# rfahrn/RadVLM

Hardware: AMD Instinct MI355X
Metric: train image-instruction pairs/sec, LLaVA-1.5-7B 336px (higher is better)
Workload: dtype bf16; 1 GPU; llava15_7b full fine-tune step (ViT frozen): fwd+bwd+AdamW, S=704, 32 pairs/GPU/step; global_batch=32, seq_len=704, parallelism=dp1, rows_with_a_label_only=last layer's o_proj / norm / MLP, final norm, lm_head, cross entropy

## Files before the change

radvlm_amd/csrc/gemm_bf16.hip:

```cpp
#include <type_traits>
#include "common.h"
#include "radvlm_hip.h"
#include "gemm_plan.h"
#include <stdlib.h>

namespace {

constexpr int BM = 128, BN = 128, BK = 64;
constexpr int STAGE_BYTES = (BM + BN) * BK * 2;
constexpr int NSTAGE = 2;

struct GemmParams {
    const bf16* A; const bf16* B; void* C; const bf16* bias; const void* R; const bf16* zeros;
    long lda, ldb, ldc, ldr;
    int M, N, K, act, out_f32, res_f32, tiles_m, tiles_n;
    float alpha;
    const bf16* A2; const bf16* B2; long lda2, ldb2; int K2;
    float* ws; int splits;
    int n_full;
    int pgrid;
    const float* rope_cs; const int* rope_pos; int rope_S, rope_cols, rope_hd;
    int F; bf16* C2; long ldc2; const bf16* G; long ldg;
    unsigned bytesA, bytesB;
    unsigned bytesA2, bytesB2;
// ... 532 lines not shown
                if (full) {
                    const f32x4 r0 = *(const f32x4*)rp, r1 = *(const f32x4*)(rp + 4);
#pragma unroll
                    for (int r = 0; r < 4; ++r) { v[r] += r0[r]; v[4 + r] += r1[r]; }
                } else {
#pragma unroll
                    for (int r = 0; r < 8; ++r) if (r < nv) v[r] += rp[r];
                }
            } else {
                const bf16* rp = (const bf16*)P.R + (long)m * P.ldr + n;
                if (full) {
                    const bf16x8 rr = *(const bf16x8*)rp;
#pragma unroll
                    for (int r = 0; r < 8; ++r) v[r] += bf2f(rr[r]);
                } else {
#pragma unroll
                    for (int r = 0; r < 8; ++r) if (r < nv) v[r] += bf2f(rp[r]);
                }
            }
        }
        if (P.out_f32) {
            float* cp = (float*)P.C + (long)m * P.ldc + n;
            if (full) { *(f32x4*)cp = f32x4{v[0], v[1], v[2], v[3]}; *(f32x4*)(cp + 4) = f32x4{v[4], v[5], v[6], v[7]}; }
            else {
#pragma unroll
                for (int r = 0; r < 8; ++r) if (r < nv) cp[r] = v[r];
            }
        } else {
            bf16* cp = (bf16*)P.C + (long)m * P.ldc + n;
            if (full) *(bf16x8*)cp = bf16x8{f2bf(v[0]), f2bf(v[1]), f2bf(v[2]), f2bf(v[3]), f2bf(v[4]), f2bf(v[5]), f2bf(v[6]), f2bf(v[7])};
            else {
#pragma unroll
                for (int r = 0; r < 8; ++r) if (r < nv) cp[r] = f2bf(v[r]);
            }
        }
    });
}

DEVINL float rbf16(float x) { return bf2f(f2bf(x)); }
DEVINL void store8(bf16* p, const float (&v)[8]) {
    *(bf16x8*)p = bf16x8{f2bf(v[0]), f2bf(v[1]), f2bf(v[2]), f2bf(v[3]), f2bf(v[4]), f2bf(v[5]), f2bf(v[6]), f2bf(v[7])};
}

template <int EPI>
DEVINL void epilogue_fused(const f32x4 (&acc)[8][4], const GemmParams& P, int m0, int tn, int wr, int wc, int lane) {
    const int q = lane >> 4;
    static_for<8>([&](auto ii) {
        constexpr int i = decltype(ii)::value;
        const int m = m0 + wr * 128 + i * 16 + (lane & 15);
        if (m >= P.M) return;
        float lo[8] = {acc[i][0][0], acc[i][0][1], acc[i][0][2], acc[i][0][3], acc[i][1][0], acc[i][1][1], acc[i][1][2], acc[i][1][3]};
        float hi[8] = {acc[i][2][0], acc[i][2][1], acc[i][2][2], acc[i][2][3], acc[i][3][0], acc[i][3][1], acc[i][3][2], acc[i][3][3]};
        if (EPI == EPI_ROPE) {
            const int half = P.rope_hd >> 1;
            int nlo, e0;
            if (P.rope_hd == 128) { e0 = 32 * (wc & 1) + 8 * q; nlo = tn * BN2 + (wc >> 1) * 128 + e0; }
            else { e0 = 8 * q; nlo = tn * BN2 + wc * 64 + e0; }
            const int nhi = nlo + half;
            if (nlo >= P.N) return;
            if (P.bias) {
                const bf16x8 b0 = *(const bf16x8*)(P.bias + nlo), b1 = *(const bf16x8*)(P.bias + nhi);
#pragma unroll
                for (int r = 0; r < 8; ++r) { lo[r] += bf2f(b0[r]); hi[r] += bf2f(b1[r]); }
            }
            if (nlo < P.rope_cols) {
                const int pos = P.rope_pos ? P.rope_pos[m] : (m % P.rope_S);
                const float* cs = P.rope_cs + ((long)pos * half + e0) * 2;
#pragma unroll
                for (int r4 = 0; r4 < 4; ++r4) {
                    const f32x4 t = *(const f32x4*)(cs + 4 * r4);
#pragma unroll
                    for (int u = 0; u < 2; ++u) {
                        const int r = 2 * r4 + u;
                        const float co = t[2 * u], si = t[2 * u + 1];
                        const float a = rbf16(lo[r]), b = rbf16(hi[r]);
                        lo[r] = a * co - b * si;
                        hi[r] = b * co + a * si;
                    }
                }
            }
            bf16* cp = (bf16*)P.C + (long)m * P.ldc;
            store8(cp + nlo, lo);
            store8(cp + nhi, hi);
        } else if (EPI == EPI_SWIGLU_FWD) {
            const int f = tn * 128 + 32 * wc + 8 * q;
            if (f >= P.F) return;
            float a[8];
#pragma unroll
            for (int r = 0; r < 8; ++r) {
                const float g = rbf16(lo[r]), u = rbf16(hi[r]);
                a[r] = rbf16(g / (1.f + __expf(-g))) * u;
            }
            bf16* gp = (bf16*)P.C + (long)m * P.ldc;
            store8(gp + f, lo);
            store8(gp + P.F + f, hi);
            store8(P.C2 + (long)m * P.ldc2 + f, a);
        }
    });
    if (EPI == EPI_SWIGLU_BWD) {
        auto dswiglu = [&](const f32x4& x0, const f32x4& x1, const bf16x8& gv, const bf16x8& uv, bf16* cp_g, bf16* cp_u) {
            const float da[8] = {x0[0], x0[1], x0[2], x0[3], x1[0], x1[1], x1[2], x1[3]};
            float dg[8], du[8];
#pragma unroll
            for (int r = 0; r < 8; ++r) {
                const float g = bf2f(gv[r]), u = bf2f(uv[r]), d = rbf16(da[r]);
                const float sg = __builtin_amdgcn_rcpf(1.f + __expf(-g));
                du[r] = d * (g * sg);
                dg[r] = d * u * (sg * (1.f + g * (1.f - sg)));
            }
            store8(cp_g, dg);
            store8(cp_u, du);
        };
        if (m0 + BM2 <= P.M && tn * BN2 + BN2 <= P.F) {
            const bf16* gp = P.G + (long)(m0 + wr * 128 + (lane & 15)) * P.ldg + tn * BN2 + wc * 64 + 8 * q;
            bf16* cp = (bf16*)P.C + (long)(m0 + wr * 128 + (lane & 15)) * P.ldc + tn * BN2 + wc * 64 + 8 * q;
            bf16x8 gq[2][4], uq[2][4];
            auto fetch = [&](int bi, bf16x8 (&gd)[4], bf16x8 (&ud)[4]) {
#pragma unroll
                for (int u = 0; u < 4; ++u) {
                    const int ia = bi * 4 + u, i = ia >> 1, a = ia & 1;
                    const bf16* p = gp + (long)i * 16 * P.ldg + 32 * a;
                    gd[u] = *(const bf16x8*)p;
                    ud[u] = *(const bf16x8*)(p + P.F);
                }
            };
            fetch(0, gq[0], uq[0]);
            static_for<4>([&](auto bt) {
                constexpr int bi = decltype(bt)::value;
                if constexpr (bi + 1 < 4) fetch(bi + 1, gq[(bi + 1) & 1], uq[(bi + 1) & 1]);
                static_for<4>([&](auto ut) {
                    constexpr int u = decltype(ut)::value, ia = bi * 4 + u, i = ia >> 1, a = ia & 1;
                    bf16* c = cp + (long)i * 16 * P.ldc + 32 * a;
                    dswiglu(acc[i][2 * a], acc[i][2 * a + 1], gq[bi & 1][u], uq[bi & 1][u], c, c + P.F);
                });
            });
            return;
        }
        static_for<16>([&](auto ia) {
            constexpr int i = decltype(ia)::value >> 1, a = decltype(ia)::value & 1;
            const int m = m0 + wr * 128 + i * 16 + (lane & 15);
            const int n = tn * BN2 + wc * 64 + 32 * a + 8 * q;
            if (m >= P.M || n >= P.F) return;
            const bf16x8 gv = *(const bf16x8*)(P.G + (long)m * P.ldg + n), uv = *(const bf16x8*)(P.G + (long)m * P.ldg + P.F + n);
            bf16* cp = (bf16*)P.C + (long)m * P.ldc;
            dswiglu(acc[i][2 * a], acc[i][2 * a + 1], gv, uv, cp + n, cp + P.F + n);
        });
    }
}

#ifdef RV_STAMPS
static long long* g_stamp_host = nullptr;
extern "C" int rv_debug_set_stamp_buffer(void* p) { g_stamp_host = (long long*)p; return 0; }
#define RV_STAMP(i) do { if (MODE == 0 && P.ws && threadIdx.x == 0) ((long long*)P.ws)[(long)blockIdx.x * 4 + (i)] = wall_clock64(); } while (0)
#else
#define RV_STAMP(i) do { } while (0)
#endif

template <bool TA, bool TB, int MODE, int EPI = EPI_NONE, bool BUF = false>
__global__ __launch_bounds__(512, 1) void gemm_kernel_256(GemmParams P) {
    extern __shared__ __attribute__((aligned(16))) char smem[];
    const int wid = wave_id(), lane = lane_id();
    const int wr = wid >> 2, wc = wid & 3;
    RV_STAMP(0);

    const int nwg = P.tiles_m * P.tiles_n;
    constexpr bool PERSIST = (MODE == 0 || MODE == 1 || MODE == 3) && BUF;
    int vtile = blockIdx.x, kslice = 0;
    bool sliced = MODE == 2;
    if (MODE == 2) { vtile = (int)blockIdx.x / P.splits; kslice = (int)blockIdx.x % P.splits; }
    if (MODE == 3 && (int)blockIdx.x >= (PERSIST ? P.pgrid : P.n_full)) {
        const int r = (int)blockIdx.x - (PERSIST ? P.pgrid : P.n_full);
        vtile = P.n_full + r / P.splits; kslice = r % P.splits; sliced = true;
    }
    int m0, n0, tn;
    auto coords = [&](int vt) {
        const int pid = xcd_remap(vt, nwg);
        constexpr int GROUP_M = RV_GROUP_M;
        const int per_group = GROUP_M * P.tiles_n;
        const int group = pid / per_group;
        const int first_m = group * GROUP_M;
        const int gsz = min(P.tiles_m - first_m, GROUP_M);
        tn = (pid % per_group) / gsz;
        m0 = (first_m + (pid % per_group) % gsz) * BM2;
        n0 = tn * BN2;
    };
    coords(vtile);

    f32x4 acc[8][4];

    const int nt1 = (P.K + BK - 1) / BK;
    const int t0 = sliced ? (int)((long)kslice * nt1 / P.splits) : 0;
    const int nt = sliced ? (int)((long)(kslice + 1) * nt1 / P.splits) - t0 : (MODE == 1 ? nt1 + (P.K2 + BK - 1) / BK : nt1);
    __amdgpu_buffer_rsrc_t rsA, rsB;
    HalfPlan plA[2], plB[2];
    if constexpr (BUF) {
        rsA = __builtin_amdgcn_make_buffer_rsrc((void*)P.A, 0, P.bytesA, 0x00020000);
        rsB = __builtin_amdgcn_make_buffer_rsrc((void*)P.B, 0, P.bytesB, 0x00020000);
    }
    auto make_plans = [&]() {
#pragma unroll
        for (int h = 0; h < 2; ++h) {
            plA[h] = plan_half<TA, false, 0>(P.lda, m0 + h * 128, P.M, wid, lane, h, 0, P.bytesA);
            if (EPI == EPI_ROPE) plB[h] = P.rope_hd == 128 ? plan_half<TB, true, 1>(P.ldb, n0 + h * 128, P.N, wid, lane, h, 0, P.bytesB)
                                                            : plan_half<TB, true, 0>(P.ldb, n0 + h * 128, P.N, wid, lane, h, 0, P.bytesB);
            else if (EPI == EPI_SWIGLU_FWD) plB[h] = plan_half<TB, true, 2>(P.ldb, tn * 128, P.N, wid, lane, h, P.F, P.bytesB);
            else plB[h] = plan_half<TB, true, 0>(P.ldb, n0 + h * 128, P.N, wid, lane, h, 0, P.bytesB);
        }
    };
    __amdgpu_buffer_rsrc_t rsA2, rsB2;
    HalfPlan plA2[2], plB2[2];
    if constexpr (BUF && MODE == 1) {
        rsA2 = __builtin_amdgcn_make_buffer_rsrc((void*)P.A2, 0, P.bytesA2, 0x00020000);
        rsB2 = __builtin_amdgcn_make_buffer_rsrc((void*)P.B2, 0, P.bytesB2, 0x00020000);
    }
    auto make_plans2 = [&]() {
#pragma unroll
        for (int h = 0; h < 2; ++h) {
            plA2[h] = plan_half<TA, false, 0>(P.lda2, m0 + h * 128, P.M, wid, lane, h, 0, P.bytesA2);
            plB2[h] = plan_half<TB, true, 0>(P.ldb2, n0 + h * 128, P.N, wid, lane, h, 0, P.bytesB2);
        }
    };
    if constexpr (BUF) make_plans();
    if constexpr (BUF && MODE == 1) make_plans2();
    const int kstepA = TA ? (int)(P.lda * BK * 2) : BK * 2, kstepB = TB ? (int)(P.ldb * BK * 2) : BK * 2;
    const int kstepA2 = TA ? (int)(P.lda2 * BK * 2) : BK * 2, kstepB2 = TB ? (int)(P.ldb2 * BK * 2) : BK * 2;
    auto stageA = [&](int t, int slot, int h, auto pair_tag) {
        constexpr int PAIR = decltype(pair_tag)::value;
        char* dst = smem + (slot * 2 + h) * HALF_BYTES;
        if constexpr (BUF) {
            if (MODE == 1 && (PAIR == 1 || (PAIR == 2 && t >= nt1))) stage_half_buf(rsA2, plA2[h], (t - nt1) * kstepA2, dst, wid);
            else stage_half_buf(rsA, plA[h], (t0 + t) * kstepA, dst, wid);
            return;
        }
        if (MODE == 1 && t >= nt1) stage_half<TA>(P.A2, P.lda2, m0 + h * 128, P.M, (t - nt1) * BK, P.K2, P.zeros, dst, wid, lane);
        else stage_half<TA>(P.A, P.lda, m0 + h * 128, P.M, (t0 + t) * BK, P.K, P.zeros, dst, wid, lane);
    };
    auto stageB = [&](int t, int h, auto pair_tag) {
        constexpr int PAIR = decltype(pair_tag)::value;
        char* dst = smem + B_RING_OFF + ((t & 1) * 2 + h) * HALF_BYTES;
        if constexpr (BUF) {
            if (MODE == 1 && (PAIR == 1 || (PAIR == 2 && t >= nt1))) stage_half_buf(rsB2, plB2[h], (t - nt1) * kstepB2, dst, wid);
            else stage_half_buf(rsB, plB[h], (t0 + t) * kstepB, dst, wid);
            return;
        }
        if (MODE == 1 && t >= nt1) stage_half<TB, true>(P.B2, P.ldb2, n0 + h * 128, P.N, (t - nt1) * BK, P.K2, P.zeros, dst, wid, lane);
        else if (EPI == EPI_ROPE) {
            if (P.rope_hd == 128) stage_half<TB, true, 1>(P.B, P.ldb, n0 + h * 128, P.N, (t0 + t) * BK, P.K, P.zeros, dst, wid, lane);
            else stage_half<TB, true>(P.B, P.ldb, n0 + h * 128, P.N, (t0 + t) * BK, P.K, P.zeros, dst, wid, lane);
        } else if (EPI == EPI_SWIGLU_FWD) stage_half<TB, true, 2>(P.B, P.ldb, tn * 128, P.N, (t0 + t) * BK, P.K, P.zeros, dst, wid, lane, h, P.F);
        else stage_half<TB, true>(P.B, P.ldb, n0 + h * 128, P.N, (t0 + t) * BK, P.K, P.zeros, dst, wid, lane);
    };

    constexpr std::integral_constant<int, 0> P0{};
    constexpr std::integral_constant<int, 1> P1{};
    constexpr std::integral_constant<int, 2> PR{};
    stageA(0, 0, 0, P0); stageA(0, 0, 1, P0); stageB(0, 0, P0); stageB(0, 1, P0);
    int vt0 = blockIdx.x;
    do {
    if (nt > 1) { stageA(1, 1, 0, PR); stageA(1, 1, 1, PR); stageB(1, 0, PR); stageB(1, 1, PR); asm volatile("s_waitcnt vmcnt(8)" ::: "memory"); }
    else asm volatile("s_waitcnt vmcnt(0)" ::: "memory");
    __builtin_amdgcn_s_barrier();
    RV_STAMP(1);
#pragma unroll
    for (int i = 0; i < 8; ++i)
#pragma unroll
        for (int j = 0; j < 4; ++j) acc[i][j] = f32x4{0.f, 0.f, 0.f, 0.f};

    int aslot = 0;
    long long dbg[4] = {0, 0, 0, 0};
    auto step = [&](int t, auto stage_tag, auto pair_tag) {
        constexpr int STAGE = decltype(stage_tag)::value;
        const char* At = smem + (aslot * 2 + wr) * HALF_BYTES;
        const char* Bt = smem + B_RING_OFF + ((t & 1) * 2 + (wc >> 1)) * HALF_BYTES;
        const int aslot2 = aslot == 0 ? 2 : aslot - 1;
        const int brow0 = (wc & 1) * 64;
        ktile_256<TA, TB>(acc, At, Bt, brow0, lane,
                          [&]() { if (STAGE == 1 || (STAGE == 2 && t + 2 < nt)) stageA(t + 2, aslot2, 0, pair_tag); },
                          [&]() { if (STAGE == 1 || (STAGE == 2 && t + 2 < nt)) stageA(t + 2, aslot2, 1, pair_tag); },
                          [&]() { if (STAGE == 1 || (STAGE == 2 && t + 2 < nt)) stageB(t + 2, 0, pair_tag); },
                          [&]() { if (STAGE == 1 || (STAGE == 2 && t + 2 < nt)) stageB(t + 2, 1, pair_tag); }, dbg);
        RV_ACC_BEGIN();
        if (STAGE == 1 || (STAGE == 2 && t + 2 < nt)) asm volatile("s_waitcnt vmcnt(8)" ::: "memory");
        else asm volatile("s_waitcnt vmcnt(0)" ::: "memory");
        RV_ACC_END(1);
        aslot = aslot == 2 ? 0 : aslot + 1;
        RV_ACC_BEGIN();
        BAR_LGKM();
        RV_ACC_END(2);
    };
    if constexpr ((MODE == 2 || MODE == 1) && !BUF) {
        for (int t = 0; t < nt; ++t) step(t, std::integral_constant<int, 2>{}, PR);
    } else if constexpr (MODE == 1) {
        int t = 0;
        for (; t + 2 < nt1; ++t) step(t, std::integral_constant<int, 1>{}, P0);
        for (; t + 2 < nt; ++t) step(t, std::integral_constant<int, 1>{}, P1);
        for (; t < nt; ++t) step(t, std::integral_constant<int, 0>{}, P0);
    } else {
        int t = 0;
        for (; t + 2 < nt; ++t) step(t, std::integral_constant<int, 1>{}, P0);
        for (; t < nt; ++t) step(t, std::integral_constant<int, 0>{}, P0);
    }
#ifdef RV_STAMPS
    if (MODE == 0 && P.ws && lane == 0) {
        long long* o = (long long*)P.ws + (long)gridDim.x * 4 + ((long)blockIdx.x * 8 + wid) * 3;
        o[0] = dbg[0]; o[1] = dbg[1]; o[2] = dbg[2];
    }
#endif

    RV_STAMP(2);
    if (MODE == 3 && sliced) {
        float* slab = P.ws + ((long)(vtile - P.n_full) * P.splits + kslice) * (BM2 * BN2);
#pragma unroll
        for (int i = 0; i < 8; ++i)
#pragma unroll
            for (int a = 0; a < 2; ++a) {
                float* wp = slab + (wr * 128 + i * 16 + (lane & 15)) * BN2 + wc * 64 + 32 * a + 8 * (lane >> 4);
                *(f32x4*)wp = acc[i][2 * a];
                *(f32x4*)(wp + 4) = acc[i][2 * a + 1];
            }
        return;
    }
    const int m0e = m0, n0e = n0, tne = tn;
    bool more = false;
    if constexpr (PERSIST) {
        vt0 += MODE == 3 ? P.pgrid : (int)gridDim.x;
        more = !sliced && vt0 < (MODE == 3 ? P.n_full : nwg);
        if (more) {
            coords(vt0); make_plans();
            if constexpr (MODE == 1) make_plans2();
            stageA(0, 0, 0, P0); stageA(0, 0, 1, P0); stageB(0, 0, P0); stageB(0, 1, P0);
        }
    }
    if (EPI != EPI_NONE) epilogue_fused<EPI>(acc, P, m0e, tne, wr, wc, lane);
    else epilogue_256<MODE == 3 ? 0 : MODE>(acc, P, m0e, n0e, wr, wc, lane, kslice);
#ifdef RV_STAMPS
    asm volatile("s_waitcnt vmcnt(0)" ::: "memory");
#endif
    RV_STAMP(3);
    if (!more) break;
    } while (PERSIST);
}

__global__ void splitk_reduce_kernel(GemmParams P) {
    const long i = (long)blockIdx.x * blockDim.x + threadIdx.x;
    const long total = (long)P.M * P.N;
    if (i >= total) return;
    const int m = (int)(i / P.N), n = (int)(i % P.N);
    float s = 0.f;
    for (int k = 0; k < P.splits; ++k) s += P.ws[(long)k * total + i];
    s *= P.alpha;
    if (P.bias) s += bf2f(P.bias[n]);
    s = apply_act(s, P.act);
    if (P.R) s += P.res_f32 ? ((const float*)P.R)[(long)m * P.ldr + n] : bf2f(((const bf16*)P.R)[(long)m * P.ldr + n]);
    if (P.out_f32) ((float*)P.C)[(long)m * P.ldc + n] = s;
    else ((bf16*)P.C)[(long)m * P.ldc + n] = f2bf(s);
}

constexpr int AG_BM = 64, AG_BN = 128;
constexpr int AG_XB = AG_BM * AG_BN * 2, AG_TB = AG_BM * 64 * 2, AG_STAGE = AG_XB + AG_TB;
struct LoraAGradParams {
    const bf16* X; const bf16* T; float* ws;
    long ldx, ldt;
    int M, R, K, splits;
    unsigned thr; unsigned long long seed;
};
DEVINL int sw128(int m) { return (((m >> 1) & 1) | (((m >> 3) & 1) << 1)) << 1; }
DEVINL bf16x8 tr_read16(const char* a, const char* b) {
    const s16x4 lo = __builtin_amdgcn_ds_read_tr16_b64_v4i16((__attribute__((address_space(3))) s16x4*)a);
    const s16x4 hi = __builtin_amdgcn_ds_read_tr16_b64_v4i16((__attribute__((address_space(3))) s16x4*)b);
    const s16x8 r = {lo[0], lo[1], lo[2], lo[3], hi[0], hi[1], hi[2], hi[3]};
    return __builtin_bit_cast(bf16x8, r);
}
__global__ __launch_bounds__(256, 3) void lora_agrad_kernel(LoraAGradParams P) {
    __shared__ __attribute__((aligned(16))) char smem[2 * AG_STAGE];
    const int wid = wave_id(), lane = lane_id(), tid = (int)threadIdx.x;
    const int ncb = (P.K + AG_BN - 1) / AG_BN;
    const int cb = (int)blockIdx.x % ncb, split = (int)blockIdx.x / ncb;
    const int c0 = cb * AG_BN;
    const int nst = (P.M + AG_BM - 1) / AG_BM;
    const int s0 = (int)((long)split * nst / P.splits), s1 = (int)((long)(split + 1) * nst / P.splits);
    const int xr = tid >> 4, xc = tid & 15;
    const int tr = tid >> 3, tc = tid & 7;
    const bool xok = c0 + xc * 8 < P.K, tok = tc * 8 < P.R;
    const bf16x8 zero8 = {0, 0, 0, 0, 0, 0, 0, 0};
    bf16x8 xv0, xv1, xv2, xv3, tv0, tv1;
    auto ldx8 = [&](int m) __attribute__((always_inline)) { return (xok && m < P.M) ? *(const bf16x8*)(P.X + (long)m * P.ldx + c0 + xc * 8) : zero8; };
    auto ldt8 = [&](int m) __attribute__((always_inline)) { return (tok && m < P.M) ? *(const bf16x8*)(P.T + (long)m * P.ldt + tc * 8) : zero8; };
    auto load = [&](int s) __attribute__((always_inline)) {
        const int m0 = s * AG_BM;
        xv0 = ldx8(m0 + xr); xv1 = ldx8(m0 + xr + 16); xv2 = ldx8(m0 + xr + 32); xv3 = ldx8(m0 + xr + 48);
        tv0 = ldt8(m0 + tr); tv1 = ldt8(m0 + tr + 32);
    };
    auto put_x = [&](bf16x8 v, int m0, int row, char* st) __attribute__((always_inline)) {
        if (P.thr) {
            const unsigned keep = rv_keep8(P.seed, (unsigned long long)(m0 + row) * (unsigned long long)P.K + (unsigned long long)(c0 + xc * 8), P.thr);
#pragma unroll
            for (int j = 0; j < 8; ++j) v[j] = (keep >> j) & 1 ? v[j] : (bf16)0.f;
        }
        *(bf16x8*)(st + row * 256 + ((xc ^ tswz(row)) << 4)) = v;
    };
    auto store = [&](int s, char* st) __attribute__((always_inline)) {
        const int m0 = s * AG_BM;
        put_x(xv0, m0, xr, st); put_x(xv1, m0, xr + 16, st); put_x(xv2, m0, xr + 32, st); put_x(xv3, m0, xr + 48, st);
        *(bf16x8*)(st + AG_XB + tr * 128 + ((tc ^ sw128(tr)) << 4)) = tv0;
        *(bf16x8*)(st + AG_XB + (tr + 32) * 128 + ((tc ^ sw128(tr + 32)) << 4)) = tv1;
    };
    const int g = lane >> 4, q = (lane >> 2) & 3, pp = lane & 3;
    const int mrow = 8 * g + q;
    int xoff[2], toff[4];
#pragma unroll
    for (int j = 0; j < 2; ++j) xoff[j] = mrow * 256 + (((((wid * 32 + 16 * j) >> 3) + (pp >> 1)) ^ tswz(mrow)) << 4) + (pp & 1) * 8;
#pragma unroll
    for (int i = 0; i < 4; ++i) toff[i] = AG_XB + mrow * 128 + ((((16 * i) >> 3) + (pp >> 1)) ^ sw128(mrow)) * 16 + (pp & 1) * 8;
    f32x4 acc[4][2];
#pragma unroll
    for (int i = 0; i < 4; ++i)
#pragma unroll
        for (int j = 0; j < 2; ++j) acc[i][j] = f32x4{0.f, 0.f, 0.f, 0.f};
    if (s0 < s1) { load(s0); store(s0, smem); }
    __syncthreads();
    for (int s = s0; s < s1; ++s) {
        const char* cur = smem + ((s - s0) & 1) * AG_STAGE;
        char* nxt = smem + (((s - s0) & 1) ^ 1) * AG_STAGE;
        if (s + 1 < s1) load(s + 1);
#pragma unroll
        for (int kk = 0; kk < 2; ++kk) {
            bf16x8 b[2], a[4];
#pragma unroll
            for (int j = 0; j < 2; ++j) b[j] = tr_read16(cur + xoff[j] + kk * 8192, cur + xoff[j] + kk * 8192 + 1024);
#pragma unroll
            for (int i = 0; i < 4; ++i) a[i] = tr_read16(cur + toff[i] + kk * 4096, cur + toff[i] + kk * 4096 + 512);
#pragma unroll
            for (int i = 0; i < 4; ++i)
#pragma unroll
                for (int j = 0; j < 2; ++j) acc[i][j] = mfma16(a[i], b[j], acc[i][j]);
        }
        if (s + 1 < s1) store(s + 1, nxt);
        __syncthreads();
    }
#pragma unroll
    for (int i = 0; i < 4; ++i)
#pragma unroll
        for (int j = 0; j < 2; ++j)
#pragma unroll
            for (int r = 0; r < 4; ++r) {
                const int ar = 16 * i + 4 * g + r, col = c0 + wid * 32 + 16 * j + (lane & 15);
                if (ar < P.R && col < P.K) P.ws[((long)split * P.R + ar) * P.K + col] = acc[i][j][r];
            }
}

__global__ __launch_bounds__(256) void tail_reduce_kernel(GemmParams P) {
    const int nwg = P.tiles_m * P.tiles_n;
    const int tt = blockIdx.x >> 5;
    const int e = ((blockIdx.x & 31) * 256 + threadIdx.x) * 8;
    const int row = e >> 8, col = e & 255;
    const int pid = xcd_remap(P.n_full + tt, nwg);
    constexpr int GROUP_M = RV_GROUP_M;
    const int per_group = GROUP_M * P.tiles_n;
    const int group = pid / per_group;
    const int first_m = group * GROUP_M;
    const int gsz = min(P.tiles_m - first_m, GROUP_M);
    const int m = (first_m + (pid % per_group) % gsz) * BM2 + row;
    const int n = ((pid % per_group) / gsz) * BN2 + col;
    if (m >= P.M || n >= P.N) return;
    float v[8] = {0, 0, 0, 0, 0, 0, 0, 0};
    for (int k = 0; k < P.splits; ++k) {
        const float* sp = P.ws + ((long)tt * P.splits + k) * (BM2 * BN2) + row * BN2 + col;
        const f32x4 a = *(const f32x4*)sp, b = *(const f32x4*)(sp + 4);
#pragma unroll
        for (int r = 0; r < 4; ++r) { v[r] += a[r]; v[4 + r] += b[r]; }
    }
    const int nv = min(8, P.N - n);
    const bool vec = nv == 8 && (P.N % 8 == 0) && (P.ldc % 8 == 0) && !P.out_f32 && (!P.R || (!P.res_f32 && P.ldr % 8 == 0)) &&
                     ((((uintptr_t)P.C) | ((uintptr_t)P.R) | ((uintptr_t)P.bias)) & 15) == 0;
    if (vec) {
        float x[8];
#pragma unroll
        for (int r = 0; r < 8; ++r) x[r] = v[r] * P.alpha;
        if (P.bias) {
            const bf16x8 bb = *(const bf16x8*)(P.bias + n);
#pragma unroll
            for (int r = 0; r < 8; ++r) x[r] += bf2f(bb[r]);
        }
        if (P.act != RV_ACT_NONE) {
#pragma unroll
            for (int r = 0; r < 8; ++r) x[r] = apply_act(x[r], P.act);
        }
        if (P.R) {
            const bf16x8 rr = *(const bf16x8*)((const bf16*)P.R + (long)m * P.ldr + n);
#pragma unroll
            for (int r = 0; r < 8; ++r) x[r] += bf2f(rr[r]);
        }
// ... 12 lines not shown

}

static_assert(PLAN_TILE128 == BM && PLAN_TILE128 == BN && PLAN_TILE256 == BM2 && PLAN_TILE256 == BN2 && PLAN_BK == BK, "gemm_plan.h plans for these tiles");
static GemmConfig g_cfg;
static int g_cus_device = -1;
static int g_reserved_cus = -1;
extern "C" int rv_gemm_select_kernel(int which) {
    if (which >= 40) g_cfg.persist = which == 41;
    else if (which >= 30) g_cfg.flat = which == 30;
    else if (which >= 20) g_cfg.tail_split = which - 20;
    else g_cfg.force_kernel = which;
    return RV_OK;
}
extern "C" int rv_gemm_set_cu_budget(int total_cus, int reserved_cus) {
    int dev = -1;
    if (hipGetDevice(&dev) != hipSuccess) dev = -1;
    if (total_cus <= 0 && (dev < 0 || hipDeviceGetAttribute(&total_cus, hipDeviceAttributeMultiprocessorCount, dev) != hipSuccess)) return RV_ERR_LAUNCH;
    g_cus_device = dev;
    g_reserved_cus = reserved_cus < 0 ? 0 : reserved_cus;
    g_cfg.cus = total_cus - g_reserved_cus < 8 ? 8 : total_cus - g_reserved_cus;
    return g_cfg.cus;
}
static int gemm_config(GemmConfig& cfg) {
    static bool env_read = false;
    if (const char* e = env_read ? nullptr : getenv("RV_GEMM_KERNEL")) g_cfg.force_kernel = atoi(e);
    env_read = true;
    int dev = 0;
    if (g_cfg.cus != 0 && hipGetDevice(&dev) == hipSuccess && dev != g_cus_device) g_cfg.cus = 0;
    if (g_cfg.cus == 0) {
        const char* e = getenv("RV_GEMM_RESERVED_CUS");
        const int rc = rv_gemm_set_cu_budget(0, g_reserved_cus >= 0 ? g_reserved_cus : (e ? atoi(e) : 0));
        if (rc < 0) return rc;
    }
    cfg = g_cfg;
    return RV_OK;
}

static GemmParams gemm_params(const void* A, int64_t lda, const void* B, int64_t ldb, void* C, int64_t ldc, const void* bias, const void* residual,
                              int64_t ldr, const void* zeros16, int M, int N, int K, float alpha, int act = RV_ACT_NONE, int out_f32 = 0, int res_f32 = 0) {
    GemmParams P = {};
    P.A = (const bf16*)A; P.B = (const bf16*)B; P.C = C; P.bias = (const bf16*)bias; P.R = residual; P.zeros = (const bf16*)zeros16;
    P.lda = lda; P.ldb = ldb; P.ldc = ldc; P.ldr = ldr;
    P.M = M; P.N = N; P.K = K; P.act = act; P.out_f32 = out_f32; P.res_f32 = res_f32; P.alpha = alpha; P.splits = 1;
    return P;
}
static void launch_splitk_reduce(const GemmParams& P, hipStream_t st) {
    hipLaunchKernelGGL(splitk_reduce_kernel, dim3((unsigned)(((long)P.M * P.N + 255) / 256)), dim3(256), 0, st, P);
}
template <bool TA, bool TB, int MODE, int EPI, bool BUF>
static void launch256(GemmParams P, const GemmPlan& pl, hipStream_t st) {
    static bool attr = false;
    if (!attr) { (void)hipFuncSetAttribute((const void*)gemm_kernel_256<TA, TB, MODE, EPI, BUF>, hipFuncAttributeMaxDynamicSharedMemorySize, LDS_BYTES2); attr = true; }
    P.tiles_m = pl.tiles_m; P.tiles_n = pl.tiles_n; P.splits = pl.splits; P.n_full = pl.n_full; P.pgrid = pl.pgrid;
    P.bytesA = pl.bytesA; P.bytesB = pl.bytesB; P.bytesA2 = pl.bytesA2; P.bytesB2 = pl.bytesB2;
    hipLaunchKernelGGL((gemm_kernel_256<TA, TB, MODE, EPI, BUF>), dim3(pl.grid), dim3(512), LDS_BYTES2, st, P);
    if (MODE == 3) hipLaunchKernelGGL(tail_reduce_kernel, dim3((pl.tiles_m * pl.tiles_n - pl.n_full) * 32), dim3(256), 0, st, P);
    if (MODE == 2) launch_splitk_reduce(P, st);
}
template <class F>
static void with_bool(bool v, F f) { if (v) f(std::true_type{}); else f(std::false_type{}); }
static void launch256_plain(const GemmParams& P, const GemmPlan& pl, bool trans_a, bool trans_b, hipStream_t st) {
    with_bool(trans_a, [&](auto ta) { with_bool(trans_b, [&](auto tb) { with_bool(pl.buf != 0, [&](auto buf) {
        constexpr bool TA = decltype(ta)::value, TB = decltype(tb)::value, BUF = decltype(buf)::value;
        switch (pl.mode) {
            case 1: launch256<TA, TB, 1, EPI_NONE, BUF>(P, pl, st); break;
            case 2: launch256<TA, TB, 2, EPI_NONE, BUF>(P, pl, st); break;
            case 3: launch256<TA, TB, 3, EPI_NONE, BUF>(P, pl, st); break;
            default: launch256<TA, TB, 0, EPI_NONE, BUF>(P, pl, st);
        }
    }); }); });
}

static int gemm_ex_impl(const void* A, int64_t lda, const void* B, int64_t ldb, void* C, int64_t ldc, const void* bias,
                        const void* residual, int64_t ldr, int M, int N, int K, int trans_a, int trans_b, float alpha,
                        int act, int out_f32, int res_f32, const void* A2, int64_t lda2, const void* B2, int64_t ldb2,
                        int K2, void* workspace, int64_t workspace_bytes, const void* zeros16, void* stream, float drop_p, uint64_t drop_seed) {
    const bool ext = A2 && B2 && K2 > 0;
    const unsigned drop_thr = drop_p > 0.f ? rv_dropout_thr16(drop_p) : 0u;
    const GemmRequest rq = {M, N, K, trans_a, trans_b, lda, ldb, ext ? K2 : 0, lda2, ldb2, workspace && workspace_bytes > 0 ? workspace_bytes : 0,
                            drop_thr ? GEMM_DROPOUT : GEMM_PLAIN};
    if (!A || !B || !C || !zeros16 || !gemm_args_ok(rq)) return RV_ERR_ARG;
    if (((uintptr_t)A | (uintptr_t)B | (uintptr_t)zeros16) & 15) return RV_ERR_ARG;
    if (ext && (((uintptr_t)A2 | (uintptr_t)B2) & 15)) return RV_ERR_ARG;
    GemmConfig cfg;
    if (const int rc = gemm_config(cfg)) return rc;
    GemmParams P = gemm_params(A, lda, B, ldb, C, ldc, bias, residual, ldr, zeros16, M, N, K, alpha, act, out_f32, res_f32);
    P.A2 = (const bf16*)A2; P.B2 = (const bf16*)B2; P.lda2 = lda2; P.ldb2 = ldb2; P.K2 = rq.K2; P.ws = (float*)workspace;
    P.drop_thr = drop_thr; P.drop_scale = drop_p > 0.f ? 1.f / (1.f - drop_p) : 1.f; P.drop_seed = drop_seed;
    const GemmPlan pl = gemm_plan(rq, cfg);
    hipStream_t st = (hipStream_t)stream;
    if (pl.use256) {
#ifdef RV_STAMPS
        if (pl.mode == 0) P.ws = (float*)g_stamp_host;
#endif
        launch256_plain(P, pl, trans_a, trans_b, st);
    } else {
        static bool attr = false;
        if (!attr) { (void)hipFuncSetAttribute((const void*)gemm_nt_kernel, hipFuncAttributeMaxDynamicSharedMemorySize, NSTAGE * STAGE_BYTES); attr = true; }
        P.tiles_m = pl.tiles_m; P.tiles_n = pl.tiles_n;
        hipLaunchKernelGGL(gemm_nt_kernel, dim3(pl.grid), dim3(256), NSTAGE * STAGE_BYTES, st, P);
    }
    return rv_check_launch();
}

extern "C" int rv_gemm_bf16_ex(const void* A, int64_t lda, const void* B, int64_t ldb, void* C, int64_t ldc, const void* bias,
                               const void* residual, int64_t ldr, int M, int N, int K, int trans_a, int trans_b, float alpha,
                               int act, int out_f32, int res_f32, const void* A2, int64_t lda2, const void* B2, int64_t ldb2,
                               int K2, void* workspace, int64_t workspace_bytes, const void* zeros16, void* stream) {
    return gemm_ex_impl(A, lda, B, ldb, C, ldc, bias, residual, ldr, M, N, K, trans_a, trans_b, alpha, act, out_f32, res_f32, A2, lda2, B2, ldb2, K2,
                        workspace, workspace_bytes, zeros16, stream, 0.f, 0);
}

extern "C" int rv_gemm_plan(int M, int N, int K, int trans_a, int trans_b, int64_t lda, int64_t ldb, int K2, int64_t lda2, int64_t ldb2,
                            int64_t workspace_bytes, int kind, int32_t* out) {
    const GemmRequest rq = {M, N, K, trans_a, trans_b, lda, ldb, K2, lda2, ldb2, workspace_bytes, kind};
    if (!out || !gemm_args_ok(rq)) return RV_ERR_ARG;
    GemmConfig cfg;
    if (const int rc = gemm_config(cfg)) return rc;
    const GemmPlan pl = gemm_plan(rq, cfg);
    out[0] = pl.use256 ? 2 : 1; out[1] = pl.mode; out[2] = pl.splits; out[3] = pl.n_full; out[4] = pl.grid; out[5] = pl.buf;
    return RV_OK;
}

extern "C" int rv_gemm_dropout_add_bf16(const void* A, int64_t lda, const void* B, int64_t ldb, void* C, int64_t ldc, int M, int N, int K,
                                        int trans_b, float alpha, float p, uint64_t seed, int accumulate, const void* zeros16, void* stream) {
    if (p < 0.f || p >= 1.f || (N & 7) || (ldc & 7) || (((uintptr_t)C) & 15)) return RV_ERR_ARG;
    return gemm_ex_impl(A, lda, B, ldb, C, ldc, nullptr, accumulate ? C : nullptr, ldc, M, N, K, 0, trans_b, alpha, RV_ACT_NONE, 0, 0, nullptr, 0,
                        nullptr, 0, 0, nullptr, 0, zeros16, stream, p, seed);
}

extern "C" int rv_gemm_bf16(const void* A, int64_t lda, const void* B, int64_t ldb, void* C, int64_t ldc, const void* bias,
                            const void* residual, int64_t ldr, int M, int N, int K, int trans_a, int trans_b, float alpha,
                            int act, int out_f32, int res_f32, const void* zeros16, void* stream) {
    return rv_gemm_bf16_ex(A, lda, B, ldb, C, ldc, bias, residual, ldr, M, N, K, trans_a, trans_b, alpha, act, out_f32, res_f32,
                           nullptr, 0, nullptr, 0, 0, nullptr, 0, zeros16, stream);
}

extern "C" int rv_gemm_nt_bf16(const void* A, int64_t lda, const void* B, int64_t ldb, void* C, int64_t ldc,
                               const void* bias, const void* residual, int64_t ldr, int M, int N, int K, int act,
                               int out_f32, int res_f32, const void* zeros16, void* stream) {
    return rv_gemm_bf16(A, lda, B, ldb, C, ldc, bias, residual, ldr, M, N, K, 0, 0, 1.0f, act, out_f32, res_f32, zeros16, stream);
}

static int fused_plan(int M, int N, int K, int trans_b, int64_t lda, int64_t ldb, GemmPlan& pl) {
    const GemmRequest rq = {M, N, K, 0, trans_b, lda, ldb, 0, 0, 0, 0, GEMM_FUSED};
    GemmConfig cfg;
    if (const int rc = gemm_config(cfg)) return rc;
    pl = gemm_plan(rq, cfg);
    if (!gemm_args_ok(rq)) pl.use256 = 0;
    return RV_OK;
}
template <int EPI, bool TB>
static int launch_fused(const GemmParams& P, const GemmPlan& pl, void* stream) {
    if (((uintptr_t)P.A | (uintptr_t)P.B | (uintptr_t)P.zeros) & 15) return RV_ERR_ARG;
    if (pl.buf) launch256<false, TB, 0, EPI, true>(P, pl, (hipStream_t)stream);
    else launch256<false, TB, 0, EPI, false>(P, pl, (hipStream_t)stream);
    return rv_check_launch();
}

extern "C" int rv_gemm_rope_bf16(const void* A, int64_t lda, const void* B, int64_t ldb, void* C, int64_t ldc, const void* bias,
                                 int M, int N, int K, const float* cos_sin, const int32_t* positions, int S, int rope_heads, int hd,
                                 void* workspace, int64_t workspace_bytes, const void* zeros16, void* stream) {
    if (!A || !B || !C || !cos_sin || !zeros16 || M <= 0 || N <= 0 || K <= 0 || rope_heads <= 0 || (long)rope_heads * hd > N) return RV_ERR_ARG;
    if ((hd & 15) || (!positions && S <= 0)) return RV_ERR_ARG;
    GemmPlan pl;
    if (const int rc = fused_plan(M, N, K, 0, lda, ldb, pl)) return rc;
    const bool fused = pl.use256 && (hd == 128 || hd == 64) && (N % 8 == 0) && (ldc % 8 == 0) && (N % hd == 0) &&
                       ((((uintptr_t)C) | ((uintptr_t)bias) | ((uintptr_t)cos_sin)) & 15) == 0;
    if (!fused) {
        int rc = rv_gemm_bf16_ex(A, lda, B, ldb, C, ldc, bias, nullptr, 0, M, N, K, 0, 0, 1.f, RV_ACT_NONE, 0, 0, nullptr, 0, nullptr, 0, 0,
                                 workspace, workspace_bytes, zeros16, stream);
        if (rc != RV_OK) return rc;
        return positions ? rv_rope_inplace_pos(C, ldc, cos_sin, positions, M, rope_heads, hd, 1, 1, stream)
                         : rv_rope_inplace(C, ldc, cos_sin, M, S, rope_heads, hd, 1, 1, stream);
    }
    GemmParams P = gemm_params(A, lda, B, ldb, C, ldc, bias, nullptr, 0, zeros16, M, N, K, 1.f);
    P.rope_cs = cos_sin; P.rope_pos = positions; P.rope_S = S > 0 ? S : 1; P.rope_cols = rope_heads * hd; P.rope_hd = hd;
    return launch_fused<EPI_ROPE, false>(P, pl, stream);
}

extern "C" int rv_gemm_swiglu_fwd_bf16(const void* A, int64_t lda, const void* Wgu, int64_t ldb, void* GU, int64_t ldgu, void* ACT,
                                       int64_t ldact, int M, int F, int K, void* workspace, int64_t workspace_bytes, const void* zeros16,
                                       void* stream) {
    if (!A || !Wgu || !GU || !ACT || !zeros16 || M <= 0 || F <= 0 || K <= 0 || (F & 7) || (ldgu & 7) || (ldact & 7)) return RV_ERR_ARG;
    GemmPlan pl;
    if (const int rc = fused_plan(M, 2 * F, K, 0, lda, ldb, pl)) return rc;
    if (!pl.use256 || ((((uintptr_t)GU) | ((uintptr_t)ACT)) & 15)) {
        int rc = rv_gemm_bf16_ex(A, lda, Wgu, ldb, GU, ldgu, nullptr, nullptr, 0, M, 2 * F, K, 0, 0, 1.f, RV_ACT_NONE, 0, 0, nullptr, 0, nullptr,
                                 0, 0, workspace, workspace_bytes, zeros16, stream);
        if (rc != RV_OK) return rc;
        return rv_swiglu_fwd(GU, ldgu, ACT, ldact, M, F, stream);
    }
    GemmParams P = gemm_params(A, lda, Wgu, ldb, GU, ldgu, nullptr, nullptr, 0, zeros16, M, 2 * F, K, 1.f);
    P.F = F; P.C2 = (bf16*)ACT; P.ldc2 = ldact;
    return launch_fused<EPI_SWIGLU_FWD, false>(P, pl, stream);
}

extern "C" int rv_gemm_swiglu_bwd_bf16(const void* dY, int64_t ldy, const void* Wd, int64_t ldw, const void* GU, int64_t ldgu, void* dGU,
                                       int64_t lddgu, void* dact_scratch, int64_t ld_dact, int M, int F, int K, void* workspace,
                                       int64_t workspace_bytes, const void* zeros16, void* stream) {
    if (!dY || !Wd || !GU || !dGU || !zeros16 || M <= 0 || F <= 0 || K <= 0 || (F & 7) || (ldgu & 7) || (lddgu & 7)) return RV_ERR_ARG;
    GemmPlan pl;
    if (const int rc = fused_plan(M, F, K, 1, ldy, ldw, pl)) return rc;
    if (!pl.use256 || ((((uintptr_t)GU) | ((uintptr_t)dGU)) & 15)) {
        if (!dact_scratch || (ld_dact & 7)) return RV_ERR_ARG;
        int rc = rv_gemm_bf16_ex(dY, ldy, Wd, ldw, dact_scratch, ld_dact, nullptr, nullptr, 0, M, F, K, 0, 1, 1.f, RV_ACT_NONE, 0, 0, nullptr, 0,
                                 nullptr, 0, 0, workspace, workspace_bytes, zeros16, stream);
        if (rc != RV_OK) return rc;
        return rv_swiglu_bwd(dact_scratch, ld_dact, GU, ldgu, dGU, lddgu, M, F, stream);
    }
    GemmParams P = gemm_params(dY, ldy, Wd, ldw, dGU, lddgu, nullptr, nullptr, 0, zeros16, M, F, K, 1.f);
    P.F = F; P.G = (const bf16*)GU; P.ldg = ldgu;
    return launch_fused<EPI_SWIGLU_BWD, true>(P, pl, stream);
}

extern "C" int rv_lora_a_grad_bf16(const void* dT, int64_t ldt, const void* X, int64_t ldx, void* gA, int64_t ldg, int M, int R, int K, float p,
                                   uint64_t seed, int accumulate, void* workspace, int64_t workspace_bytes, void* stream) {
    if (!dT || !X || !gA || !workspace || M <= 0 || R <= 0 || K <= 0 || p < 0.f || p >= 1.f) return RV_ERR_ARG;
    if (R > 64 || (R & 7) || (K & 7) || (ldx & 7) || (ldt & 7) || (p > 0.f && ldx != K)) return RV_ERR_ARG;
    if ((((uintptr_t)X) | ((uintptr_t)dT)) & 15) return RV_ERR_ARG;
    const int ncb = (K + AG_BN - 1) / AG_BN, nst = (M + AG_BM - 1) / AG_BM;
    GemmConfig cfg;
    if (const int rc = gemm_config(cfg)) return rc;
    int splits = (3 * cfg.cus + ncb - 1) / ncb;
    if (splits > nst) splits = nst;
    if (splits > 32) splits = 32;
    const int64_t per = (int64_t)R * K * 4;
    if (splits > workspace_bytes / per) splits = (int)(workspace_bytes / per);
    if (splits < 1) return RV_ERR_ARG;
    LoraAGradParams Q;
    Q.X = (const bf16*)X; Q.T = (const bf16*)dT; Q.ws = (float*)workspace; Q.ldx = ldx; Q.ldt = ldt; Q.M = M; Q.R = R; Q.K = K; Q.splits = splits;
    Q.thr = rv_dropout_thr16(p); Q.seed = seed;
    hipStream_t st = (hipStream_t)stream;
    hipLaunchKernelGGL(lora_agrad_kernel, dim3((unsigned)(ncb * splits)), dim3(256), 0, st, Q);
    GemmParams P = gemm_params(nullptr, 0, nullptr, 0, gA, ldg, nullptr, accumulate ? gA : nullptr, ldg, nullptr, R, K, 0, p > 0.f ? 1.f / (1.f - p) : 1.f);
    P.splits = splits; P.ws = (float*)workspace;
    launch_splitk_reduce(P, st);
    return rv_check_launch();
}

extern "C" int rv_lora_down_bf16(const void* X, int64_t ldx, const void* A, int64_t lda, void* T, int64_t ldt, int M, int R, int K, float alpha,
                                 float p, uint64_t seed, const void* zeros16, void* stream) {
    if (!X || !A || !T || !zeros16 || M <= 0 || R <= 0 || K <= 0 || p < 0.f || p >= 1.f) return RV_ERR_ARG;
    if (R > LD_BN || (R & 3) || (K % BK) || (p > 0.f && ldx != K) || (ldx & 7) || (lda & 7) || (ldt & 3)) return RV_ERR_ARG;
    if ((((uintptr_t)X) | ((uintptr_t)A) | ((uintptr_t)zeros16)) & 15) return RV_ERR_ARG;
    if (((uintptr_t)T) & 7) return RV_ERR_ARG;
    static bool attr = false;
    if (!attr) { (void)hipFuncSetAttribute((const void*)lora_down_kernel, hipFuncAttributeMaxDynamicSharedMemorySize, LD_NSTAGE * LD_STAGE); attr = true; }
    LoraDownParams P;
    P.X = (const bf16*)X; P.A = (const bf16*)A; P.T = (bf16*)T; P.zeros = (const bf16*)zeros16;
    P.ldx = ldx; P.lda = lda; P.ldt = ldt; P.M = M; P.R = R; P.K = K;
    P.alpha = p > 0.f ? alpha / (1.f - p) : alpha;
    P.thr = rv_dropout_thr16(p); P.seed = seed;
    hipLaunchKernelGGL(lora_down_kernel, dim3((M + LD_BM - 1) / LD_BM), dim3(256), LD_NSTAGE * LD_STAGE, (hipStream_t)stream, P);
    return rv_check_launch();
}
```

Baseline: 40.38 pairs/s.

## Carry next persistent tile's prologue loads across the tile seam in GEMM

In the persistent 256-tile GEMM kernel (MODE 0/3 with buffered loads), the last two k-steps of a tile now prefetch the first two k-tiles of the next tile. This overlaps the next tile's global loads with the current tile's tail compute and epilogue instead of restarting the pipeline after each epilogue. A/B slot and parity now rotate continuously across tiles rather than being reset. Plans for the next tile are computed mid-loop; when no tile follows, plans point at out-of-range offsets so the loads become no-ops. It also adds seam timing stamps under RV_STAMPS, which adds register and control complexity.

```diff
diff --git a/radvlm_amd/csrc/gemm_bf16.hip b/radvlm_amd/csrc/gemm_bf16.hip
--- a/radvlm_amd/csrc/gemm_bf16.hip
+++ b/radvlm_amd/csrc/gemm_bf16.hip
@@ -708,8 +708,19 @@
 static long long* g_stamp_host = nullptr;
 extern "C" int rv_debug_set_stamp_buffer(void* p) { g_stamp_host = (long long*)p; return 0; }
 #define RV_STAMP(i) do { if (MODE == 0 && P.ws && threadIdx.x == 0) ((long long*)P.ws)[(long)blockIdx.x * 4 + (i)] = wall_clock64(); } while (0)
+#define RV_SEAM_TILES 32
+#define RV_SEAM_SLOT(k, i) ((long long*)P.ws)[(long)gridDim.x * 28 + ((long)blockIdx.x * RV_SEAM_TILES + (k)) * 8 + (i)]
+#define RV_SEAM_ON(k) (MODE == 0 && PERSIST && P.ws && threadIdx.x == 0 && (k) >= 0 && (k) < RV_SEAM_TILES)
+#define RV_SEAM(i) do { const int k_ = (i) >= 3 ? seam_i - 1 : seam_i; if (RV_SEAM_ON(k_)) RV_SEAM_SLOT(k_, i) = wall_clock64(); } while (0)
+#define RV_SEAM_PLAN_BEGIN() do { if (RV_SEAM_ON(seam_i)) RV_SEAM_SLOT(seam_i, 5) = wall_clock64(); } while (0)
+#define RV_SEAM_PLAN_END() do { if (RV_SEAM_ON(seam_i)) RV_SEAM_SLOT(seam_i, 6) = wall_clock64(); } while (0)
+#define RV_SEAM_NEXT() do { if (RV_SEAM_ON(seam_i)) RV_SEAM_SLOT(seam_i, 7) = nt; ++seam_i; } while (0)
 #else
 #define RV_STAMP(i) do { } while (0)
+#define RV_SEAM(i) do { } while (0)
+#define RV_SEAM_PLAN_BEGIN() do { } while (0)
+#define RV_SEAM_PLAN_END() do { } while (0)
+#define RV_SEAM_NEXT() do { } while (0)
 #endif
 
 template <bool TA, bool TB, int MODE, int EPI = EPI_NONE, bool BUF = false>
@@ -791,9 +802,9 @@
         if (MODE == 1 && t >= nt1) stage_half<TA>(P.A2, P.lda2, m0 + h * 128, P.M, (t - nt1) * BK, P.K2, P.zeros, dst, wid, lane);
         else stage_half<TA>(P.A, P.lda, m0 + h * 128, P.M, (t0 + t) * BK, P.K, P.zeros, dst, wid, lane);
     };
-    auto stageB = [&](int t, int h, auto pair_tag) {
+    auto stageB = [&](int t, int par, int h, auto pair_tag) {
         constexpr int PAIR = decltype(pair_tag)::value;
-        char* dst = smem + B_RING_OFF + ((t & 1) * 2 + h) * HALF_BYTES;
+        char* dst = smem + B_RING_OFF + (par * 2 + h) * HALF_BYTES;
         if constexpr (BUF) {
             if (MODE == 1 && (PAIR == 1 || (PAIR == 2 && t >= nt1))) stage_half_buf(rsB2, plB2[h], (t - nt1) * kstepB2, dst, wid);
             else stage_half_buf(rsB, plB[h], (t0 + t) * kstepB, dst, wid);
@@ -810,51 +821,87 @@
     constexpr std::integral_constant<int, 0> P0{};
     constexpr std::integral_constant<int, 1> P1{};
     constexpr std::integral_constant<int, 2> PR{};
-    stageA(0, 0, 0, P0); stageA(0, 0, 1, P0); stageB(0, 0, P0); stageB(0, 1, P0);
+    stageA(0, 0, 0, P0); stageA(0, 0, 1, P0); stageB(0, 0, 0, P0); stageB(0, 0, 1, P0);
     int vt0 = blockIdx.x;
+    int aslot = 0, bpar = 0;
+    constexpr bool CARRY = PERSIST && MODE != 1;
+    bool carried = false;
+#ifdef RV_STAMPS
+    int seam_i = 0;
+#endif
     do {
-    if (nt > 1) { stageA(1, 1, 0, PR); stageA(1, 1, 1, PR); stageB(1, 0, PR); stageB(1, 1, PR); asm volatile("s_waitcnt vmcnt(8)" ::: "memory"); }
-    else asm volatile("s_waitcnt vmcnt(0)" ::: "memory");
-    __builtin_amdgcn_s_barrier();
+    if (!carried) {
+        if (nt > 1) {
+            const int s1 = aslot == 2 ? 0 : aslot + 1;
+            stageA(1, s1, 0, PR); stageA(1, s1, 1, PR); stageB(1, bpar ^ 1, 0, PR); stageB(1, bpar ^ 1, 1, PR);
+            asm volatile("s_waitcnt vmcnt(8)" ::: "memory");
+        } else asm volatile("s_waitcnt vmcnt(0)" ::: "memory");
+        __builtin_amdgcn_s_barrier();
+    }
     RV_STAMP(1);
+    RV_SEAM(3);
 #pragma unroll
     for (int i = 0; i < 8; ++i)
 #pragma unroll
         for (int j = 0; j < 4; ++j) acc[i][j] = f32x4{0.f, 0.f, 0.f, 0.f};
 
-    int aslot = 0;
+    const int m0e = m0, n0e = n0, tne = tn;
+    bool more = false;
+    int vnext = 0;
+    if constexpr (PERSIST) {
+        vnext = vt0 + (MODE == 3 ? P.pgrid : (int)gridDim.x);
+        more = !sliced && vnext < (MODE == 3 ? P.n_full : nwg);
+    }
+    carried = false;
     long long dbg[4] = {0, 0, 0, 0};
-    auto step = [&](int t, auto stage_tag, auto pair_tag) {
+    auto step = [&](int ts, auto stage_tag, auto pair_tag) {
         constexpr int STAGE = decltype(stage_tag)::value;
         const char* At = smem + (aslot * 2 + wr) * HALF_BYTES;
-        const char* Bt = smem + B_RING_OFF + ((t & 1) * 2 + (wc >> 1)) * HALF_BYTES;
+        const char* Bt = smem + B_RING_OFF + (bpar * 2 + (wc >> 1)) * HALF_BYTES;
         const int aslot2 = aslot == 0 ? 2 : aslot - 1;
         const int brow0 = (wc & 1) * 64;
         ktile_256<TA, TB>(acc, At, Bt, brow0, lane,
-                          [&]() { if (STAGE == 1 || (STAGE == 2 && t + 2 < nt)) stageA(t + 2, aslot2, 0, pair_tag); },
-                          [&]() { if (STAGE == 1 || (STAGE == 2 && t + 2 < nt)) stageA(t + 2, aslot2, 1, pair_tag); },
-                          [&]() { if (STAGE == 1 || (STAGE == 2 && t + 2 < nt)) stageB(t + 2, 0, pair_tag); },
-                          [&]() { if (STAGE == 1 || (STAGE == 2 && t + 2 < nt)) stageB(t + 2, 1, pair_tag); }, dbg);
+                          [&]() { if (STAGE == 1 || (STAGE == 2 && ts < nt)) stageA(ts, aslot2, 0, pair_tag); },
+                          [&]() { if (STAGE == 1 || (STAGE == 2 && ts < nt)) stageA(ts, aslot2, 1, pair_tag); },
+                          [&]() { if (STAGE == 1 || (STAGE == 2 && ts < nt)) stageB(ts, bpar, 0, pair_tag); },
+                          [&]() { if (STAGE == 1 || (STAGE == 2 && ts < nt)) stageB(ts, bpar, 1, pair_tag); }, dbg);
         RV_ACC_BEGIN();
-        if (STAGE == 1 || (STAGE == 2 && t + 2 < nt)) asm volatile("s_waitcnt vmcnt(8)" ::: "memory");
+        if (STAGE == 1 || (STAGE == 2 && ts < nt)) asm volatile("s_waitcnt vmcnt(8)" ::: "memory");
         else asm volatile("s_waitcnt vmcnt(0)" ::: "memory");
         RV_ACC_END(1);
         aslot = aslot == 2 ? 0 : aslot + 1;
+        bpar ^= 1;
         RV_ACC_BEGIN();
         BAR_LGKM();
         RV_ACC_END(2);
     };
     if constexpr ((MODE == 2 || MODE == 1) && !BUF) {
-        for (int t = 0; t < nt; ++t) step(t, std::integral_constant<int, 2>{}, PR);
+        for (int t = 0; t < nt; ++t) step(t + 2, std::integral_constant<int, 2>{}, PR);
     } else if constexpr (MODE == 1) {
         int t = 0;
-        for (; t + 2 < nt1; ++t) step(t, std::integral_constant<int, 1>{}, P0);
-        for (; t + 2 < nt; ++t) step(t, std::integral_constant<int, 1>{}, P1);
-        for (; t < nt; ++t) step(t, std::integral_constant<int, 0>{}, P0);
+        for (; t + 2 < nt1; ++t) step(t + 2, std::integral_constant<int, 1>{}, P0);
+        for (; t + 2 < nt; ++t) step(t + 2, std::integral_constant<int, 1>{}, P1);
+        for (; t < nt; ++t) step(0, std::integral_constant<int, 0>{}, P0);
+    } else if constexpr (CARRY) {
+        int t = 0;
+#ifdef RV_STAMPS
+        if (nt > 2) { step(2, std::integral_constant<int, 1>{}, P0); t = 1; RV_SEAM(4); }
+#endif
+        for (; t + 2 < nt; ++t) step(t + 2, std::integral_constant<int, 1>{}, P0);
+        RV_SEAM_PLAN_BEGIN();
+        if (more && nt >= 2) { coords(vnext); make_plans(); carried = true; }
+        else {
+#pragma unroll
+            for (int h = 0; h < 2; ++h)
+#pragma unroll
+                for (int i = 0; i < 2; ++i) { plA[h].v[i] = (int)P.bytesA; plB[h].v[i] = (int)P.bytesB; }
+        }
+        RV_SEAM_PLAN_END();
+        for (; t < nt; ++t) step(t + 2 - nt, std::integral_constant<int, 1>{}, P0);
     } else {
         int t = 0;
-        for (; t + 2 < nt; ++t) step(t, std::integral_constant<int, 1>{}, P0);
-        for (; t < nt; ++t) step(t, std::integral_constant<int, 0>{}, P0);
+        for (; t + 2 < nt; ++t) step(t + 2, std::integral_constant<int, 1>{}, P0);
+        for (; t < nt; ++t) step(0, std::integral_constant<int, 0>{}, P0);
     }
 #ifdef RV_STAMPS
     if (MODE == 0 && P.ws && lane == 0) {
@@ -874,26 +921,29 @@
                 *(f32x4*)wp = acc[i][2 * a];
                 *(f32x4*)(wp + 4) = acc[i][2 * a + 1];
             }
+        if constexpr (CARRY) asm volatile("s_waitcnt vmcnt(0)" ::: "memory");
         return;
     }
-    const int m0e = m0, n0e = n0, tne = tn;
-    bool more = false;
+    RV_SEAM(0);
     if constexpr (PERSIST) {
-        vt0 += MODE == 3 ? P.pgrid : (int)gridDim.x;
-        more = !sliced && vt0 < (MODE == 3 ? P.n_full : nwg);
-        if (more) {
+        vt0 = vnext;
+        if (more && !carried) {
             coords(vt0); make_plans();
             if constexpr (MODE == 1) make_plans2();
-            stageA(0, 0, 0, P0); stageA(0, 0, 1, P0); stageB(0, 0, P0); stageB(0, 1, P0);
-        }
-    }
+            stageA(0, aslot, 0, P0); stageA(0, aslot, 1, P0); stageB(0, bpar, 0, P0); stageB(0, bpar, 1, P0);
+        }
+    }
+    RV_SEAM(1);
     if (EPI != EPI_NONE) epilogue_fused<EPI>(acc, P, m0e, tne, wr, wc, lane);
     else epilogue_256<MODE == 3 ? 0 : MODE>(acc, P, m0e, n0e, wr, wc, lane, kslice);
+    RV_SEAM(2);
+    if (CARRY && !more) asm volatile("s_waitcnt vmcnt(0)" ::: "memory");
 #ifdef RV_STAMPS
-    asm volatile("s_waitcnt vmcnt(0)" ::: "memory");
+    if (!more) asm volatile("s_waitcnt vmcnt(0)" ::: "memory");
 #endif
     RV_STAMP(3);
     if (!more) break;
+    RV_SEAM_NEXT();
     } while (PERSIST);
 }
 
@@ -1212,8 +1262,11 @@
     return RV_OK;
 }
 template <int EPI, bool TB>
-static int launch_fused(const GemmParams& P, const GemmPlan& pl, void* stream) {
+static int launch_fused(GemmParams P, const GemmPlan& pl, void* stream) {
     if (((uintptr_t)P.A | (uintptr_t)P.B | (uintptr_t)P.zeros) & 15) return RV_ERR_ARG;
+#ifdef RV_STAMPS
+    P.ws = (float*)g_stamp_host;
+#endif
     if (pl.buf) launch256<false, TB, 0, EPI, true>(P, pl, (hipStream_t)stream);
     else launch256<false, TB, 0, EPI, false>(P, pl, (hipStream_t)stream);
     return rv_check_launch();
```

After: 40.38 pairs/s, median of 3. No clear change (+0.0%).
